# alexfrom0815/IR-BPP

Measured on AMD Instinct MI355X. Metric: env steps/sec (placements/sec) across N parallel bins, higher is better.
Workload: dtype f64

## Files before the change

irbpp_amd/csrc/irbpp_kernels.hip:

```cpp
#include <hip/hip_runtime.h>
#include <math.h>
#include <stdint.h>

#include "contours_device.h"
#include "irbpp_device.h"
#include "irbpp_rounds.h"
#include "../../include/irbpp.h"

#ifndef IRBPP_PASS
#define IRBPP_PASS 1
#endif

#undef IRBPP_HERE
#undef IRBPP_PASS_NS
#if IRBPP_PASS == 1
#define IRBPP_HERE ::irbpp::
#elif IRBPP_PASS == 2
#define IRBPP_HERE ::irbpp::wg512::
#define IRBPP_PASS_NS wg512
#else
#define IRBPP_HERE ::irbpp::wg128::
#define IRBPP_PASS_NS wg128
#endif

namespace irbpp {
#if IRBPP_PASS != 1
namespace IRBPP_PASS_NS {
#endif

#if IRBPP_PASS == 1
constexpr int BLOCK = 256;
#elif IRBPP_PASS == 2
constexpr int BLOCK = 512;
#else
constexpr int BLOCK = 128;
#endif
constexpr int WAVES = BLOCK / 64;

#ifndef IRBPP_REPS
#ifdef IRBPP_ABLATE
#define IRBPP_REPS(bit) (1 + ((P.dbg_repeat >> (bit)) & 1))
#else
#define IRBPP_REPS(bit) 1
#endif
#endif

#if IRBPP_PASS == 1
__device__ __forceinline__ double round6(double x) { return rint(x * 1e6) / 1e6; }

__device__ __forceinline__ double round6_scaled(double x) { return rint(x * 1e6); }

__device__ __forceinline__ int np_floor_divide_int(double a, double b, double inv_b) {
    const double x = fabs(a);
    const double q0 = trunc(x * inv_b);
    const double r0 = fma(-q0, b, x);
    int q = (int)q0 + (r0 >= b ? 1 : 0) - (r0 < 0.0 ? 1 : 0);
#if defined(__HIP_DEVICE_COMPILE__)
    if (__ballot(a < 0.0) == 0ull) return q;
#endif
    if (a < 0.0) {
        const double r = fma(-(double)q, b, x);
        q = r == 0.0 ? -q : -q - 1;
    }
    return q;
}


__device__ __forceinline__ double wave_max_f64(double v) {
#define IRBPP_MAX_STEP(CTRL, ROWS)                                                                                   \
    {                                                                                                                \
        const int lo = __builtin_amdgcn_update_dpp(__double2loint(v), __double2loint(v), CTRL, ROWS, 0xF, false);    \
        const int hi = __builtin_amdgcn_update_dpp(__double2hiint(v), __double2hiint(v), CTRL, ROWS, 0xF, false);    \
        v = fmax(v, __hiloint2double(hi, lo));                                                                       \
    }
    IRBPP_MAX_STEP(0x111, 0xF) IRBPP_MAX_STEP(0x112, 0xF) IRBPP_MAX_STEP(0x114, 0xF) IRBPP_MAX_STEP(0x118, 0xF)
    IRBPP_MAX_STEP(0x142, 0xA) IRBPP_MAX_STEP(0x143, 0xC)
#undef IRBPP_MAX_STEP
    return __hiloint2double(__builtin_amdgcn_readlane(__double2hiint(v), 63), __builtin_amdgcn_readlane(__double2loint(v), 63));
}

#endif
__device__ inline double block_max_f64(double v, double* red) {
    v = wave_max_f64(v);
    __syncthreads();
    if ((threadIdx.x & 63) == 0) red[threadIdx.x >> 6] = v;
    __syncthreads();
    double r = red[0];
    for (int w = 1; w < WAVES; ++w) r = fmax(r, red[w]);
    return r;
}

__device__ inline int block_sum_int(int v, int* red) {
    v = __builtin_amdgcn_readlane(wave_inclusive_sum(v), 63);
    __syncthreads();
    if ((threadIdx.x & 63) == 0) red[threadIdx.x >> 6] = v;
    __syncthreads();
    int r = 0;
    for (int w = 0; w < WAVES; ++w) r += red[w];
    return r;
}

__device__ inline int block_scan_flag(bool flag, int* red, int& total) {
    const unsigned long long bal = __ballot(flag);
    const int lane = threadIdx.x & 63, w = threadIdx.x >> 6;
    const int pre = __popcll(bal & ((1ull << lane) - 1ull));
    __syncthreads();
    if (lane == 0) red[w] = __popcll(bal);
    __syncthreads();
    int base = 0;
    total = 0;
    for (int i = 0; i < WAVES; ++i) {
        const int c = red[i];
        if (i < w) base += c;
        total += c;
    }
    return base + pre;
}

#if IRBPP_PASS == 1
__device__ inline int trajectory_row(const Params& P, const Tables& T, int b, int episode) {
    long long row = T.stream ? (long long)b : (long long)P.traj_start + P.goff + b + (long long)episode * P.gbins;
    row %= T.n_traj;
    if (row < 0) row += T.n_traj;
    return (int)row;
}
struct KernArgs;
__device__ __forceinline__ void raise_error(const State& S, int bit);
constexpr int STREAM_CONSUMED = -3;
__device__ inline int consume_item(const Tables& T, const State& S, int row, int cursor, int id) {
    if (T.stream) {
        if (id == STREAM_CONSUMED) { raise_error(S, IRBPP_DEVERR_STREAM_DRY); return -1; }
        const_cast<int32_t*>(T.seq)[(long long)row * T.seq_len + (int)((uint32_t)cursor % (uint32_t)T.seq_len)] = STREAM_CONSUMED;
    }
    if (id >= T.n_shapes) { raise_error(S, IRBPP_DEVERR_BAD_ITEM); return -1; }
    return id < 0 ? -1 : id;
}
__device__ inline int fetch_item(const Tables& T, const State& S, int row, int cursor) {
    if (!T.stream && cursor >= T.seq_len) return -1;
    const int at = T.stream ? (int)((uint32_t)cursor % (uint32_t)T.seq_len) : cursor;
    return consume_item(T, S, row, cursor, T.seq[(long long)row * T.seq_len + at]);
}

__device__ __forceinline__ int fdiv(int n, int d, uint32_t m) {
    return d == 1 ? n : (int)__umulhi((uint32_t)n, m);
}

struct KernArgs { Params P; Tables T; State S; StepIO io; int mode; };
typedef const __attribute__((address_space(4))) KernArgs* KernArgsPtr;
__device__ __forceinline__ KernArgsPtr cold_args() {
    KernArgsPtr p = (KernArgsPtr)__builtin_amdgcn_kernarg_segment_ptr();
    asm volatile("" : "+s"(p));
    return p;
}

__device__ __forceinline__ void raise_error(const State& S, int bit) {
    atomicOr(S.err, bit);
    int32_t* mirror = cold_args()->io.err_out;
    if (mirror != nullptr) atomicOr(mirror, bit);
}

__device__ __forceinline__ uint32_t div_magic_dev(int d) { return d >= 2 ? (uint32_t)(0x100000000ull / (uint64_t)d + 1ull) : 0u; }

__device__ __forceinline__ int tile_row_part(const Params& P, int row) {
    const int q = fdiv(row, P.pp, P.mg_pp);
    return (row - q * P.pp) * P.pp * P.PL + q * P.LY;
}
__device__ __forceinline__ int tile_col_part(const Params& P, int col) {
    const int q = fdiv(col, P.pp, P.mg_pp);
    return (col - q * P.pp) * P.PL + q;
}
__device__ __forceinline__ int tile_rc(const Params& P, int row, int col) { return tile_row_part(P, row) + tile_col_part(P, col); }
__device__ __forceinline__ int tile_of_linear(const Params& P, int g) {
    const int row = fdiv(g, P.Hy, P.mg_hy);
    return tile_rc(P, row, g - row * P.Hy);
}
#endif
struct TileWalk {
    int col_part, row, row_step, lin;
    bool regular;
};
__device__ __forceinline__ TileWalk tile_walk_begin(const Params& P, int tid) {
    TileWalk w;
    const int row = fdiv(tid, P.Hy, P.mg_hy), col = tid - row * P.Hy;
    w.regular = BLOCK % P.Hy == 0;
    w.row = row;
    w.row_step = BLOCK / P.Hy;
    w.col_part = tile_col_part(P, col);
    w.lin = tid;
    return w;
}
__device__ __forceinline__ int tile_walk_index(const Params& P, const TileWalk& w) {
    return w.regular ? tile_row_part(P, w.row) + w.col_part : tile_of_linear(P, w.lin);
}
__device__ __forceinline__ void tile_walk_next(TileWalk& w) { w.lin += BLOCK; w.row += w.row_step; }
template <int STEP>
__device__ __forceinline__ void cell_tile_stage(const Params& P, double* c2, const double* ghm, float* obs, int tid) {
    if (tid >= P.AC) return;
    const int X = fdiv(tid, P.Ay, P.mg_ay), Y = tid - X * P.Ay;
    const int at = X * STEP * P.Hy + Y * STEP;
    const double* src = ghm + at;
    float* dst = obs + 5 * P.S + 9 + at;
    typedef double f64x2 __attribute__((ext_vector_type(2)));
    double h[STEP][STEP];
#pragma unroll
    for (int i = 0; i < STEP; ++i) {
        if constexpr (STEP == 1) {
            h[i][0] = src[0];
        } else {
#pragma unroll
            for (int j = 0; j < STEP; j += 2) {
                const f64x2 v = *(const f64x2*)(src + i * P.Hy + j);
                h[i][j] = v.x;
                h[i][j + 1] = v.y;
            }
        }
    }
    double m = h[0][0];
#pragma unroll
    for (int i = 0; i < STEP; ++i)
#pragma unroll
        for (int j = 0; j < STEP; ++j)
            if (i + j > 0) m = fmax(m, h[i][j]);
    c2[tid] = m;
#pragma unroll
    for (int i = 0; i < STEP; ++i)
#pragma unroll
        for (int j = 0; j < STEP; ++j) dst[i * P.Hy + j] = (float)h[i][j];
}
#if IRBPP_PASS == 1
__device__ __forceinline__ int tile_of_cell(const Params& P, int lx, int ly, int ij) {
    return tile_rc(P, lx * P.step + (ij & 0xFFFF), ly * P.step + (ij >> 16));
}

typedef const __attribute__((address_space(4))) Cell* ConstCellPtr;
__device__ __forceinline__ ConstCellPtr as_const(const Cell* p) { return (ConstCellPtr)(unsigned long long)p; }

constexpr int PHASE_ROW = 16;
__device__ __forceinline__ void stamp(const StepIO& io, int b, int k, bool leader) {
    if (io.phase_cycles && leader) {
        long long* row = io.phase_cycles + (size_t)b * PHASE_ROW;
        row[k] = (long long)clock64();
        if (k == 0) {
            row[8] = (long long)wall_clock64();
            const unsigned hw = __builtin_amdgcn_s_getreg((31 << 11) | 4);
            const unsigned xcc = __builtin_amdgcn_s_getreg((31 << 11) | 20);
            row[10] = (long long)hw | ((long long)xcc << 32);
        }
        if (k == 4) row[9] = (long long)wall_clock64();
    }
}

__device__ __forceinline__ void stamp(const StepIO& io, int b, int k) { stamp(io, b, k, threadIdx.x == 0); }

__device__ inline SlotMem carve_slot(unsigned char* base, int cap, int cap_stk) {
    SlotMem m;
    m.pts = base;
    m.dst = m.pts + cap;
    m.stk = (uint32_t*)(m.dst + cap);
    m.cap = cap;
    m.cap_stk = cap_stk;
    return m;
}

struct Lds {
    int* sr;
    double* hm;
    double* mb;
    double* c2;
    double* m1;
    double* posz;
    uint8_t* lev;
    unsigned long long* present;
    uint16_t* taskidx;
    uint16_t* tasklist;
    uint16_t* img;
    uint16_t* clist;
    uint32_t* dps;
    uint32_t* vmask;
    uint32_t* vbits;
    unsigned char* scratch;
    double* redd;
    int* redi;
};

__device__ inline Lds carve_lds(unsigned char* smem, const Params& P) {
    Lds L;
    L.sr = (int*)(smem + P.o_sr);
    L.hm = (double*)(smem + P.o_hm);
    L.mb = (double*)(smem + P.o_mb);
    L.c2 = (double*)(smem + P.o_c2);
    L.m1 = (double*)(smem + P.o_m1);
    L.posz = (double*)(smem + P.o_posz);
    L.lev = smem + P.o_lev;
// ... 2135 lines not shown
            for (int e = tid; e < s_nt; e += BLOCK) {
                const Cell tc = e == tid ? tc0 : cells[e];
                const int ij = tc.ij;
                const int row = lx * P.step + (ij & 0xFFFF), col = ly * P.step + (ij >> 16);
                const int c = tile_rc(P, row, col);
                const double h = fmax(L.hm[c], tc.v + z);
                L.hm[c] = h;
                ghm[row * P.Hy + col] = h;
            }
        } else {
            for (int i = tid; i < P.tile_words; i += BLOCK) L.hm[i] = 0.0;
            for (int i = tid; i < P.Hc; i += BLOCK) ghm[i] = 0.0;
        }
        if (tid == 0) {
            BinState* ps = S.bs + b;
            const KernArgsPtr ka = cold_args();
            if (ok) {
                const double vol = vol0;
                const double reward = (vol / P.bin_vol) * 10.0;
                const double epr = ps->ep_reward + reward;
                const int epl = ps->ep_len + 1;
                const int cursor = st_cursor;
                const int slot = ps->item_idx;
                if (ka->S.log_meta && slot < ka->S.log_cap) {
                    __builtin_assume(lx < 32 && ly < 32);
                    ka->S.log_meta[(size_t)b * ka->S.log_cap + slot] = (uint32_t)item0 | ((uint32_t)rot << 16) |
                                                                ((uint32_t)lx << 20) | ((uint32_t)ly << 25);
                    ka->S.log_z[(size_t)b * ka->S.log_cap + slot] = z;
                }
                ps->ep_reward = epr;
                ps->ep_len = epl;
                ps->item_idx += 1;
                ps->ratio_acc += vol;
                for (int i = oa; i < P.K - 1; ++i) q[i] = q[i + 1];
                int nxt = st_next;
                if (nxt == -2) nxt = fetch_item(T, S, st_trow, cursor);
                else nxt = consume_item(T, S, st_trow, cursor, nxt);
                q[P.K - 1] = nxt;
                ps->cursor = cursor + 1;
                if (ka->io.reward) ka->io.reward[b] = reward;
                if (ka->io.done) ka->io.done[b] = 0;
                if (ka->io.counter) ka->io.counter[b] = -1;
                if (ka->io.ratio) ka->io.ratio[b] = -1.0;
                if (ka->io.ep_reward) ka->io.ep_reward[b] = epr;
                if (ka->io.ep_len) ka->io.ep_len[b] = epl;
                if (ka->io.stable) ka->io.stable[b] = stable ? 1 : 0;
            } else {
                const int counter = ps->item_idx;
                const double ratio = ps->ratio_acc / P.bin_vol;
                const double epr = ps->ep_reward + 0.0;
                const int epl = ps->ep_len + 1;
                if (ka->io.stable) ka->io.stable[b] = 0;
                if (ka->io.reward) ka->io.reward[b] = 0.0;
                if (ka->io.done) ka->io.done[b] = 1;
                if (ka->io.counter) ka->io.counter[b] = counter;
                if (ka->io.ratio) ka->io.ratio[b] = ratio;
                if (ka->io.ep_reward) ka->io.ep_reward[b] = epr;
                if (ka->io.ep_len) ka->io.ep_len[b] = epl;
                if (ka->S.log_meta && counter < ka->S.log_cap) {
                    ka->S.log_meta[(size_t)b * ka->S.log_cap + counter] = (uint32_t)(item0 & 0xFFFF) | ((uint32_t)(rot & 15) << 16) |
                                                                   ((uint32_t)(lx & 31) << 20) | ((uint32_t)(ly & 31) << 25);
                    ka->S.log_z[(size_t)b * ka->S.log_cap + counter] = z;
                }
                double* tot = ka->S.totals + (size_t)b * 4;
                tot[0] += 1.0; tot[1] += ratio; tot[2] += (double)counter; tot[3] += epr;
                const int ep = ps->episode + 1;
                const int trow = trajectory_row(P, T, b, ep);
                ps->episode = ep;
                ps->traj_row = trow;
                const int c0 = T.stream ? st_cursor : 0;
                for (int i = 0; i < P.K; ++i) q[i] = fetch_item(T, S, trow, c0 + i);
                ps->cursor = c0 + P.K;
                ps->item_idx = 0;
                ps->ratio_acc = 0.0;
                ps->ep_reward = 0.0;
                ps->ep_len = 0;
            }
            for (int i = 0; i < P.K; ++i) L.redi[16 + i] = q[i];
        }
        if (ok && pref_ok) {
            if (tid < P.R * SRW_) L.sr[tid] = sr_pref;
            sr_staged = true;
        }
        __syncthreads();
    }

    if (mode == MODE_OBSERVE) stamp(io, b, 1);
    if (mode == MODE_RESET || mode == MODE_STEP) {
        stamp(io, b, 1);
        if (P.K == 1) {
            obs_item = L.redi[16];
            __syncthreads();
        } else {
            do_observe = false;
            for (int i = tid; i < P.K; i += BLOCK) obs[i] = (float)L.redi[16 + i];
            for (int i = tid; i < P.Hc; i += BLOCK) obs[P.K + i] = (float)L.hm[tile_of_linear(P, i)];
        }
    }
    if (do_observe) IRBPP_HERE observe_location<PATH, CHAIN>(P, T, S, io, L, b, obs_item, obs, debug_out, sr_staged, smem + P.lds_bytes, cell_tile);
}

#if IRBPP_PASS == 1
enum ApplyKey : int { KEY_CAND = 0, KEY_CELLS = 1, KEY_HEUR = 2 };

__device__ __forceinline__ uint32_t heuristic_select_wave(const Params& P, const State& S, int method, int dir, int b, int lane) {
    const int RAC = P.R * P.AC;
    const double* const zsrc = S.w_posz + (size_t)b * RAC;
    const uint32_t* const vsrc = S.w_valid + (size_t)b * P.R * P.vrow;
    const bool xf = (dir & 2) != 0, yf = (dir & 1) != 0;
    double best = 1e300;
    int best_i = 0x7fffffff;
    for (int i0 = 0; i0 < RAC; i0 += 4 * 64) {
        int X[4], Y[4];
        uint32_t vw[4];
        double z[4];
#pragma unroll
        for (int u = 0; u < 4; ++u) {
            const int idx = i0 + u * 64 + lane, ii = idx < RAC ? idx : 0;
            const int r = fdiv(ii, P.AC, P.mg_ac), c = ii - r * P.AC;
            X[u] = fdiv(c, P.Ay, P.mg_ay);
            Y[u] = c - X[u] * P.Ay;
            vw[u] = vsrc[r * P.vrow + X[u]];
        }
#pragma unroll
        for (int u = 0; u < 4; ++u) {
            const int idx = i0 + u * 64 + lane;
            z[u] = 1e3;
            if (idx < RAC && ((vw[u] >> Y[u]) & 1u)) z[u] = zsrc[idx];
        }
#pragma unroll
        for (int u = 0; u < 4; ++u) {
            const int idx = i0 + u * 64 + lane;
            if (idx >= RAC) continue;
            double sc = 1e6;
            if ((vw[u] >> Y[u]) & 1u) {
                const double cx = xf ? (double)(P.Ax - X[u]) : (double)X[u], cy = yf ? (double)(P.Ay - Y[u]) : (double)Y[u];
                const double raw = method == 1 ? z[u] : method == 2 ? (cx + cy) * P.res_a + 100.0 * z[u] : cx + cy;
                sc = round6(raw);
            }
            if (sc < best) { best = sc; best_i = idx; }
        }
    }
    for (int o = 32; o > 0; o >>= 1) {
        const double ob = __shfl_xor(best, o);
        const int oi = __shfl_xor(best_i, o);
        if (ob < best || (ob == best && oi < best_i)) { best = ob; best_i = oi; }
    }
    best_i = __builtin_amdgcn_readfirstlane(best_i);
    const int hr = fdiv(best_i, P.AC, P.mg_ac), hrem = best_i - hr * P.AC;
    const int hx = fdiv(hrem, P.Ay, P.mg_ay);
    return ((uint32_t)hr << 16) | ((uint32_t)hx << 8) | (uint32_t)(hrem - hx * P.Ay);
}

template <bool PER_WORKGROUP, int KEY = KEY_CAND>
__device__ __forceinline__ void apply_body(const Params& P, const Tables& T, const State& S, const StepIO& io) {
    const int lane = threadIdx.x & 63;
    const int slot = PER_WORKGROUP ? (int)blockIdx.x : (int)blockIdx.x * WAVES + (int)(threadIdx.x >> 6);
    if (slot >= io.n_slots) return;
    const int b = __builtin_amdgcn_readfirstlane(slot + io.block_off);
    double* const ghm = S.hm + (size_t)b * P.Hc;
    int32_t* const q = S.queue + (size_t)b * P.K;
    if (!PER_WORKGROUP || threadIdx.x < 64) {
    int a = 0, cell_r = 0, cell_x = 0, cell_y = 0;
    if constexpr (KEY == KEY_CAND) a = io.actions[b];
    if constexpr (KEY == KEY_CELLS) { cell_r = io.actions[3 * b]; cell_x = io.actions[3 * b + 1]; cell_y = io.actions[3 * b + 2]; }
    const BinState* ps0 = S.bs + b;
    const int item0 = ps0->cur_item, oa = ps0->order_action, nvalid0 = ps0->nvalid, nrows = ps0->nrows;
    const int cursor = ps0->cursor, trow = ps0->traj_row;
    uint32_t key;
    if constexpr (KEY == KEY_CAND) {
    a += a < 0 ? P.S : 0;
    if (a < 0 || a >= P.S) { if (lane == 0) raise_error(S, IRBPP_DEVERR_BAD_ACTION); a = a < 0 ? 0 : P.S - 1; }
    key = (uint32_t)__builtin_amdgcn_readfirstlane(a < nrows ? (int)S.cand[(size_t)b * P.S + a] : 0);
    } else if constexpr (KEY == KEY_CELLS) {
        if (cell_r < 0 || cell_r >= P.R || cell_x < 0 || cell_x >= P.Ax || cell_y < 0 || cell_y >= P.Ay) {
            if (lane == 0) raise_error(S, IRBPP_DEVERR_BAD_ACTION);
            cell_r = cell_r < 0 ? 0 : cell_r >= P.R ? P.R - 1 : cell_r;
            cell_x = cell_x < 0 ? 0 : cell_x >= P.Ax ? P.Ax - 1 : cell_x;
            cell_y = cell_y < 0 ? 0 : cell_y >= P.Ay ? P.Ay - 1 : cell_y;
        }
        key = (uint32_t)__builtin_amdgcn_readfirstlane((cell_r << 16) | (cell_x << 8) | cell_y);
        (void)nrows;
    } else {
        key = (item0 >= 0 && nvalid0 > 0) ? heuristic_select_wave(P, S, io.heur_method, io.heur_dir, b, lane) : 0u;
        (void)nrows;
    }
    int nxt = -2;
    if (P.K == 1) {
        const int at = T.stream ? (int)((uint32_t)cursor % (uint32_t)T.seq_len) : cursor;
        nxt = at < T.seq_len ? T.seq[(long long)trow * T.seq_len + at] : -1;
    }
    static_assert(sizeof(ShapeRot) == 112, "seven 16-byte chunks per ShapeRot");
    int4 srq = make_int4(0, 0, 0, 0);
    if (item0 >= 0 && lane < P.R * 7) srq = ((const int4*)(T.sr + (size_t)item0 * P.R))[lane];
    const double vol0 = item0 >= 0 ? T.volume[item0] : 0.0;
    const int rot = key >> 16, lx = (key >> 8) & 255, ly = key & 255;
    const bool have_sr = item0 >= 0 && rot < P.R;
    const int rot7 = have_sr ? rot * 7 : 0;
#define IRBPP_SRW(W) __builtin_amdgcn_readlane(((W) & 3) == 0 ? srq.x : ((W) & 3) == 1 ? srq.y : ((W) & 3) == 2 ? srq.z : srq.w, rot7 + ((W) >> 2))
#define IRBPP_SRI(FIELD) IRBPP_SRW(offsetof(ShapeRot, FIELD) / 4)
#define IRBPP_SRD(FIELD) __hiloint2double(IRBPP_SRW(offsetof(ShapeRot, FIELD) / 4 + 1), IRBPP_SRW(offsetof(ShapeRot, FIELD) / 4))
    const int s_ax = IRBPP_SRI(ax), s_ay = IRBPP_SRI(ay), s_nb = IRBPP_SRI(nb), s_ob = IRBPP_SRI(ob), s_has_out = IRBPP_SRI(has_out);
    const int s_ot = IRBPP_SRI(ot);
    const double ext_x = IRBPP_SRD(ext_x), ext_y = IRBPP_SRD(ext_y), ext_z = IRBPP_SRD(ext_z);
    bool ok = item0 >= 0 && nvalid0 > 0 && rot < P.R;
    if (ok) {
        const double tx = P.txs[lx & 31], ty = P.txs[ly & 31];
        if (round6_scaled(tx + ext_x - P.bin_x) > 0.0 || round6_scaled(ty + ext_y - P.bin_y) > 0.0) ok = false;
    }
    const int s_nt = ok ? IRBPP_SRI(nt) : 0;
#undef IRBPP_SRD
#undef IRBPP_SRI
#undef IRBPP_SRW
    const KernArgsPtr ka = cold_args();
    const bool in_grid = have_sr && lx <= P.Ax - s_ax && ly <= P.Ay - s_ay;
    const bool want_z = in_grid && (ok || ka->S.log_meta != nullptr);
    uint32_t vword = 0u;
    double zc = 1e3;
    if (want_z) {
        vword = S.w_valid[((size_t)b * P.R + rot) * P.vrow + lx];
        zc = S.w_posz[((size_t)b * P.R + rot) * P.AC + lx * P.Ay + ly];
    }
    const Cell* const tcells = T.tcell + s_ot;
    Cell tc0 = {};
    if (lane < s_nt) tc0 = tcells[lane];
    const int row0 = lx * P.step, col0 = ly * P.step;
    double h0 = 0.0;
    const int i0 = (row0 + (tc0.ij & 0xFFFF)) * P.Hy + col0 + (tc0.ij >> 16);
    if (lane < s_nt) h0 = ghm[i0];
    double z = 1e3;
    if (want_z) {
        if ((vword >> ly) & 1u) {
            z = zc;
        } else {
            const Cell* cells = T.bcell + s_ob;
            double m = s_has_out ? 0.0 : -1e300;
            for (int e = lane; e < s_nb; e += 64) {
                const Cell c = cells[e];
                m = fmax(m, ghm[(row0 + (c.ij & 0xFFFF)) * P.Hy + col0 + (c.ij >> 16)] - c.v);
            }
            z = wave_max_f64(m);
        }
    }
    if (ok) {
        const double top = z * P.scale_z + ext_z * P.scale_z;
        if (round6_scaled(top - P.ibin_z) > 0.0) ok = false;
    }
    if (ok) {
        if (lane < s_nt) ghm[i0] = fmax(h0, tc0.v + z);
        for (int e0 = 64; e0 < s_nt; e0 += 4 * 64) {
            Cell tc[4];
            int ix[4];
            double hv[4];
#pragma unroll
            for (int u = 0; u < 4; ++u) {
                const int e = e0 + u * 64 + lane;
                tc[u] = tcells[e < s_nt ? e : s_nt - 1];
            }
#pragma unroll
            for (int u = 0; u < 4; ++u) {
                ix[u] = (row0 + (tc[u].ij & 0xFFFF)) * P.Hy + col0 + (tc[u].ij >> 16);
                hv[u] = ghm[ix[u]];
            }
#pragma unroll
            for (int u = 0; u < 4; ++u)
                if (e0 + u * 64 + lane < s_nt) ghm[ix[u]] = fmax(hv[u], tc[u].v + z);
        }
    } else {
        for (int i = lane; i < P.Hc; i += 64) ghm[i] = 0.0;
    }
    if (lane == 0) {
        BinState* ps = S.bs + b;
        if (ok) {
            const double vol = vol0;
            const double reward = (vol / P.bin_vol) * 10.0;
            const double epr = ps->ep_reward + reward;
            const int epl = ps->ep_len + 1;
            const int slot_i = ps->item_idx;
            if (ka->S.log_meta && slot_i < ka->S.log_cap) {
                __builtin_assume(lx < 32 && ly < 32);
                ka->S.log_meta[(size_t)b * ka->S.log_cap + slot_i] = (uint32_t)item0 | ((uint32_t)rot << 16) |
                                                              ((uint32_t)lx << 20) | ((uint32_t)ly << 25);
                ka->S.log_z[(size_t)b * ka->S.log_cap + slot_i] = z;
            }
            ps->ep_reward = epr;
            ps->ep_len = epl;
            ps->item_idx += 1;
            ps->ratio_acc += vol;
            for (int i = oa; i < P.K - 1; ++i) q[i] = q[i + 1];
            if (nxt == -2) nxt = fetch_item(T, S, trow, cursor);
            else nxt = consume_item(T, S, trow, cursor, nxt);
            q[P.K - 1] = nxt;
            ps->cursor = cursor + 1;
            if (ka->io.reward) ka->io.reward[b] = reward;
            if (ka->io.done) ka->io.done[b] = 0;
            if (ka->io.counter) ka->io.counter[b] = -1;
            if (ka->io.ratio) ka->io.ratio[b] = -1.0;
            if (ka->io.ep_reward) ka->io.ep_reward[b] = epr;
            if (ka->io.ep_len) ka->io.ep_len[b] = epl;
            if (ka->io.stable) ka->io.stable[b] = 0;
        } else {
            const int counter = ps->item_idx;
            const double ratio = ps->ratio_acc / P.bin_vol;
            const double epr = ps->ep_reward + 0.0;
            const int epl = ps->ep_len + 1;
            if (ka->io.stable) ka->io.stable[b] = 0;
            if (ka->io.reward) ka->io.reward[b] = 0.0;
            if (ka->io.done) ka->io.done[b] = 1;
            if (ka->io.counter) ka->io.counter[b] = counter;
            if (ka->io.ratio) ka->io.ratio[b] = ratio;
            if (ka->io.ep_reward) ka->io.ep_reward[b] = epr;
            if (ka->io.ep_len) ka->io.ep_len[b] = epl;
            if (ka->S.log_meta && counter < ka->S.log_cap) {
                ka->S.log_meta[(size_t)b * ka->S.log_cap + counter] = (uint32_t)(item0 & 0xFFFF) | ((uint32_t)(rot & 15) << 16) |
                                                               ((uint32_t)(lx & 31) << 20) | ((uint32_t)(ly & 31) << 25);
                ka->S.log_z[(size_t)b * ka->S.log_cap + counter] = z;
            }
            double* tot = ka->S.totals + (size_t)b * 4;
            tot[0] += 1.0; tot[1] += ratio; tot[2] += (double)counter; tot[3] += epr;
            const int ep = ps->episode + 1;
            const int trow2 = trajectory_row(P, T, b, ep);
            ps->episode = ep;
            ps->traj_row = trow2;
            const int c0 = T.stream ? cursor : 0;
            for (int i = 0; i < P.K; ++i) q[i] = fetch_item(T, S, trow2, c0 + i);
            ps->cursor = c0 + P.K;
            ps->item_idx = 0;
            ps->ratio_acc = 0.0;
            ps->ep_reward = 0.0;
            ps->ep_len = 0;
        }
    }
    }
    if (P.K > 1 && io.obs != nullptr) {
        __builtin_amdgcn_fence(__ATOMIC_RELEASE, "workgroup");
        if (PER_WORKGROUP) __syncthreads();
        __builtin_amdgcn_fence(__ATOMIC_ACQUIRE, "workgroup");
        float* const obs = io.obs + (size_t)b * io.obs_stride;
        const int t0 = PER_WORKGROUP ? (int)threadIdx.x : lane, stride = PER_WORKGROUP ? BLOCK : 64;
        for (int i = t0; i < P.K; i += stride) obs[i] = (float)q[i];
        for (int i0 = 0; i0 < P.Hc; i0 += 8 * stride) {
            double v[8];
#pragma unroll
            for (int u = 0; u < 8; ++u) { const int i = i0 + u * stride + t0; v[u] = ghm[i < P.Hc ? i : P.Hc - 1]; }
#pragma unroll
            for (int u = 0; u < 8; ++u) { const int i = i0 + u * stride + t0; if (i < P.Hc) obs[P.K + i] = (float)v[u]; }
        }
    }
}
extern "C" __global__ void __launch_bounds__(BLOCK)
irbpp_apply_kernel(const Params P, const Tables T, const State S, const StepIO io, const int mode) { apply_body<false>(P, T, S, io); }
extern "C" __global__ void __launch_bounds__(BLOCK)
irbpp_apply_wg_kernel(const Params P, const Tables T, const State S, const StepIO io, const int mode) { apply_body<true>(P, T, S, io); }
extern "C" __global__ void __launch_bounds__(BLOCK)
irbpp_apply_cells_kernel(const Params P, const Tables T, const State S, const StepIO io, const int mode) { apply_body<false, KEY_CELLS>(P, T, S, io); }
extern "C" __global__ void __launch_bounds__(BLOCK)
irbpp_apply_cells_wg_kernel(const Params P, const Tables T, const State S, const StepIO io, const int mode) { apply_body<true, KEY_CELLS>(P, T, S, io); }
extern "C" __global__ void __launch_bounds__(BLOCK)
irbpp_apply_heur_kernel(const Params P, const Tables T, const State S, const StepIO io, const int mode) { apply_body<false, KEY_HEUR>(P, T, S, io); }
extern "C" __global__ void __launch_bounds__(BLOCK)
irbpp_apply_heur_wg_kernel(const Params P, const Tables T, const State S, const StepIO io, const int mode) { apply_body<true, KEY_HEUR>(P, T, S, io); }

extern "C" __global__ void __launch_bounds__(1024)
irbpp_item_order_kernel(const Tables T, const State S, int N) {
    __shared__ int hist[1024];
    __shared__ int start[1024];
    const int tid = threadIdx.x;
    hist[tid] = 0;
    __syncthreads();
    constexpr int PER = 8;
    auto buckets_of = [&](int k0, int (&out)[PER]) {
        int cur[PER], row[PER], item[PER];
#pragma unroll
        for (int u = 0; u < PER; ++u) {
            const int bb = tid + (k0 + u) * 1024;
            const BinState* ps = S.bs + (bb < N ? bb : 0);
            cur[u] = ps->cursor;
            row[u] = ps->traj_row;
        }
#pragma unroll
        for (int u = 0; u < PER; ++u) {
            int c = cur[u];
            if (T.stream) c = (int)((uint32_t)c % (uint32_t)T.seq_len);
            item[u] = c < T.seq_len ? T.seq[(long long)row[u] * T.seq_len + c] : 0;
        }
#pragma unroll
        for (int u = 0; u < PER; ++u) {
            const int it = item[u] < 0 ? 0 : (item[u] >= T.n_shapes ? T.n_shapes - 1 : item[u]);
            out[u] = (int)(((long long)it * 1024) / T.n_shapes);
        }
    };
    int mine[PER];
    for (int k0 = 0; k0 * 1024 < N; k0 += PER) {
        int bk[PER];
        buckets_of(k0, bk);
#pragma unroll
        for (int u = 0; u < PER; ++u) {
            if (k0 == 0) mine[u] = bk[u];
            if (tid + (k0 + u) * 1024 < N) atomicAdd(&hist[bk[u]], 1);
        }
    }
    __syncthreads();
    if (tid < 64) {
        int v[16], sum = 0;
        for (int i = 0; i < 16; ++i) { v[i] = hist[tid * 16 + i]; sum += v[i]; }
        const int inc = wave_inclusive_sum(sum);
        int acc = inc - sum;
        for (int i = 0; i < 16; ++i) { start[tid * 16 + i] = acc; acc += v[i]; }
    }
    __syncthreads();
    const int chunk = N / NXCD;
    for (int k0 = 0; k0 * 1024 < N; k0 += PER) {
        int bk[PER];
        if (k0 == 0) {
#pragma unroll
            for (int u = 0; u < PER; ++u) bk[u] = mine[u];
        } else {
            buckets_of(k0, bk);
        }
#pragma unroll
        for (int u = 0; u < PER; ++u) {
            const int bb = tid + (k0 + u) * 1024;
            if (bb < N) {
                const int s_pos = atomicAdd(&start[bk[u]], 1);
                S.order[NXCD * (s_pos % chunk) + s_pos / chunk] = bb;
            }
        }
    }
}

extern "C" __global__ void __launch_bounds__(BLOCK)
irbpp_heuristic_kernel(const Params P, const Tables T, const State S, const StepIO io) {
    extern __shared__ __attribute__((aligned(16))) unsigned char smem[];
    const Lds L = carve_lds(smem, P);
    const int b = blockIdx.x, tid = threadIdx.x;
    const int R = P.R, AC = P.AC, Ay = P.Ay;
    const int X = fdiv(tid, Ay, P.mg_ay), Y = tid - X * Ay;
    const double* ghm = S.hm + (size_t)b * P.Hc;
    for (int i = tid; i < P.Hc; i += BLOCK) L.hm[tile_of_linear(P, i)] = ghm[i];
    __syncthreads();
    const int item = __builtin_amdgcn_readfirstlane(S.bs[b].cur_item);
    overlap_test<PATH_ANY>(P, T, S, io, L, b, item, false, L.posz, false, true);
    __syncthreads();
    double best = 1e300;
    int best_i = 0x7fffffff;
    for (int r = 0; r < R; ++r) {
        if (tid < AC) {
            double sc = 1e6;
            if (item >= 0) sc = heuristic_score(P, T, io, L, T.sr[item * R + r], r, X, Y);
            const int idx = r * AC + tid;
            if (sc < best || (sc == best && idx < best_i)) { best = sc; best_i = idx; }
        }
    }
    for (int o = 32; o > 0; o >>= 1) {
        const double ob = __shfl_xor(best, o);
        const int oi = __shfl_xor(best_i, o);
        if (ob < best || (ob == best && oi < best_i)) { best = ob; best_i = oi; }
    }
    __syncthreads();
    if ((tid & 63) == 0) { L.redd[tid >> 6] = best; L.redi[4 + (tid >> 6)] = best_i; }
    __syncthreads();
    if (tid == 0) {
        for (int w = 1; w < WAVES; ++w)
            if (L.redd[w] < best || (L.redd[w] == best && L.redi[4 + w] < best_i)) { best = L.redd[w]; best_i = L.redi[4 + w]; }
        const int hr = fdiv(best_i, AC, P.mg_ac), hrem = best_i - hr * AC;
        const int hx = fdiv(hrem, Ay, P.mg_ay);
        io.heur_out[b * 3 + 0] = hr;
        io.heur_out[b * 3 + 1] = hx;
        io.heur_out[b * 3 + 2] = hrem - hx * Ay;
    }
}

constexpr int SHOT_CHUNK = 128;
extern "C" __global__ void __launch_bounds__(BLOCK)
irbpp_shot_item_kernel(const double* verts, const int32_t* faces, int n_faces, int fx, int fy, double res, double shift,
                       double* top, double* bottom, double* mtop, double* mbot, int32_t* any_hit) {
    __shared__ double tri[SHOT_CHUNK][10];
    __shared__ int n_staged;
    const int c = blockIdx.x * BLOCK + threadIdx.x;
    const bool mine = c < fx * fy;
    const double px = (double)(c / fy) * res + shift, py = (double)(c % fy) * res + shift;
    double zmin = 1e300, zmax = -1e300;
    bool hit = false;
    for (int f0 = 0; f0 < n_faces; f0 += SHOT_CHUNK) {
        __syncthreads();
        if (threadIdx.x == 0) n_staged = 0;
        __syncthreads();
        if (threadIdx.x < SHOT_CHUNK && f0 + threadIdx.x < n_faces) {
            const int f = f0 + threadIdx.x;
            const double* a = verts + 3 * faces[3 * f + 0];
            const double* b = verts + 3 * faces[3 * f + 1];
            const double* d = verts + 3 * faces[3 * f + 2];
            const double area = (b[0] - a[0]) * (d[1] - a[1]) - (b[1] - a[1]) * (d[0] - a[0]);
            if (area != 0.0) {
                double* t = tri[atomicAdd(&n_staged, 1)];
                t[0] = a[0]; t[1] = a[1]; t[2] = a[2]; t[3] = b[0]; t[4] = b[1]; t[5] = b[2];
                t[6] = d[0]; t[7] = d[1]; t[8] = d[2]; t[9] = area;
            }
        }
        __syncthreads();
        if (mine)
            for (int k = 0; k < n_staged; ++k) {
                const double* a = tri[k];
                const double* b = a + 3;
                const double* d = a + 6;
                const double area = a[9];
                const double w0 = (b[0] - px) * (d[1] - py) - (b[1] - py) * (d[0] - px);
                const double w1 = (d[0] - px) * (a[1] - py) - (d[1] - py) * (a[0] - px);
                const double w2 = (a[0] - px) * (b[1] - py) - (a[1] - py) * (b[0] - px);
                const bool inside = area > 0.0 ? (w0 >= 0.0 && w1 >= 0.0 && w2 >= 0.0) : (w0 <= 0.0 && w1 <= 0.0 && w2 <= 0.0);
                if (!inside) continue;
// ... 130 lines not shown
```

Measured before the change: 74.22 million.

## Spread apply-kernel bin-state and queue updates across wave lanes

The apply kernel now loads the 64-byte BinState with one dword per lane and broadcasts fields through readlane. It writes back only the owned dwords in a single lane-parallel store, replacing scattered lane-0 scalar accesses. Queue shifting, episode-reset refills, totals updates and heightmap clearing are now spread across lanes (double2 stores for the clear), and the next item is prefetched unconditionally. A waves-per-EU occupancy hint is added to most apply kernels. This shortens the serial lane-0 tail, at the cost of more register pressure and more complex reset logic.

After: 73.93 million. No clear change (-0.4%).

```diff
diff --git a/irbpp_amd/csrc/irbpp_kernels.hip b/irbpp_amd/csrc/irbpp_kernels.hip
--- a/irbpp_amd/csrc/irbpp_kernels.hip
+++ b/irbpp_amd/csrc/irbpp_kernels.hip
@@ -139,6 +139,14 @@
     if (!T.stream && cursor >= T.seq_len) return -1;
     const int at = T.stream ? (int)((uint32_t)cursor % (uint32_t)T.seq_len) : cursor;
     return consume_item(T, S, row, cursor, T.seq[(long long)row * T.seq_len + at]);
+}
+__device__ __forceinline__ bool reset_by_lanes(const Tables& T, int K) { return !T.stream || K <= T.seq_len; }
+__device__ __forceinline__ int reset_fetch_lane(const Tables& T, int row, int cursor, int K, int lane) {
+    if (lane >= K || !reset_by_lanes(T, K)) return -1;
+    const int c = (T.stream ? cursor : 0) + lane;
+    if (!T.stream && c >= T.seq_len) return -1;
+    const int at = T.stream ? (int)((uint32_t)c % (uint32_t)T.seq_len) : c;
+    return T.seq[(long long)row * T.seq_len + at];
 }
 
 __device__ __forceinline__ int fdiv(int n, int d, uint32_t m) {
@@ -2580,6 +2588,7 @@
     return ((uint32_t)hr << 16) | ((uint32_t)hx << 8) | (uint32_t)(hrem - hx * P.Ay);
 }
 
+#define IRBPP_APPLY_WAVES __attribute__((amdgpu_waves_per_eu(8)))
 template <bool PER_WORKGROUP, int KEY = KEY_CAND>
 __device__ __forceinline__ void apply_body(const Params& P, const Tables& T, const State& S, const StepIO& io) {
     const int lane = threadIdx.x & 63;
@@ -2592,9 +2601,17 @@
     int a = 0, cell_r = 0, cell_x = 0, cell_y = 0;
     if constexpr (KEY == KEY_CAND) a = io.actions[b];
     if constexpr (KEY == KEY_CELLS) { cell_r = io.actions[3 * b]; cell_x = io.actions[3 * b + 1]; cell_y = io.actions[3 * b + 2]; }
-    const BinState* ps0 = S.bs + b;
-    const int item0 = ps0->cur_item, oa = ps0->order_action, nvalid0 = ps0->nvalid, nrows = ps0->nrows;
-    const int cursor = ps0->cursor, trow = ps0->traj_row;
+    static_assert(sizeof(BinState) == 64, "sixteen dwords: one per lane");
+    int32_t* const bsw = (int32_t*)(S.bs + b);
+    const int bs_in = lane < 16 ? bsw[lane] : 0;
+    const KernArgsPtr ka = cold_args();
+    uint32_t* log_meta = ka->S.log_meta;
+    int log_cap = ka->S.log_cap;
+    asm volatile("" : "+s"(log_meta), "+s"(log_cap));
+#define IRBPP_BSI(FIELD) __builtin_amdgcn_readlane(bs_in, offsetof(BinState, FIELD) / 4)
+#define IRBPP_BSD(FIELD) __hiloint2double(__builtin_amdgcn_readlane(bs_in, offsetof(BinState, FIELD) / 4 + 1), __builtin_amdgcn_readlane(bs_in, offsetof(BinState, FIELD) / 4))
+    const int item0 = IRBPP_BSI(cur_item), oa = IRBPP_BSI(order_action), nvalid0 = IRBPP_BSI(nvalid), nrows = IRBPP_BSI(nrows);
+    const int cursor = IRBPP_BSI(cursor), trow = IRBPP_BSI(traj_row);
     uint32_t key;
     if constexpr (KEY == KEY_CAND) {
     a += a < 0 ? P.S : 0;
@@ -2613,11 +2630,13 @@
         key = (item0 >= 0 && nvalid0 > 0) ? heuristic_select_wave(P, S, io.heur_method, io.heur_dir, b, lane) : 0u;
         (void)nrows;
     }
-    int nxt = -2;
-    if (P.K == 1) {
+    int nxt;
+    {
         const int at = T.stream ? (int)((uint32_t)cursor % (uint32_t)T.seq_len) : cursor;
         nxt = at < T.seq_len ? T.seq[(long long)trow * T.seq_len + at] : -1;
     }
+    int qv = 0;
+    if (P.K > 1 && lane > oa && lane < P.K) qv = q[lane];
     static_assert(sizeof(ShapeRot) == 112, "seven 16-byte chunks per ShapeRot");
     int4 srq = make_int4(0, 0, 0, 0);
     if (item0 >= 0 && lane < P.R * 7) srq = ((const int4*)(T.sr + (size_t)item0 * P.R))[lane];
@@ -2640,9 +2659,8 @@
 #undef IRBPP_SRD
 #undef IRBPP_SRI
 #undef IRBPP_SRW
-    const KernArgsPtr ka = cold_args();
     const bool in_grid = have_sr && lx <= P.Ax - s_ax && ly <= P.Ay - s_ay;
-    const bool want_z = in_grid && (ok || ka->S.log_meta != nullptr);
+    const bool want_z = in_grid && (ok || log_meta != nullptr);
     uint32_t vword = 0u;
     double zc = 1e3;
     if (want_z) {
@@ -2694,71 +2712,112 @@
             for (int u = 0; u < 4; ++u)
                 if (e0 + u * 64 + lane < s_nt) ghm[ix[u]] = fmax(hv[u], tc[u].v + z);
         }
+    } else if ((P.Hc & 1) == 0) {
+        double2* const ghm2 = (double2*)ghm;
+        for (int i = lane; i < (P.Hc >> 1); i += 64) ghm2[i] = make_double2(0.0, 0.0);
     } else {
         for (int i = lane; i < P.Hc; i += 64) ghm[i] = 0.0;
     }
-    if (lane == 0) {
-        BinState* ps = S.bs + b;
-        if (ok) {
-            const double vol = vol0;
-            const double reward = (vol / P.bin_vol) * 10.0;
-            const double epr = ps->ep_reward + reward;
-            const int epl = ps->ep_len + 1;
-            const int slot_i = ps->item_idx;
-            if (ka->S.log_meta && slot_i < ka->S.log_cap) {
+    const int episode0 = IRBPP_BSI(episode), item_idx0 = IRBPP_BSI(item_idx), ep_len0 = IRBPP_BSI(ep_len);
+    const double ratio_acc0 = IRBPP_BSD(ratio_acc), ep_reward0 = IRBPP_BSD(ep_reward);
+#undef IRBPP_BSD
+#undef IRBPP_BSI
+    double* const log_z = ka->S.log_z;
+    double* const totals = ka->S.totals;
+    double* const o_reward = ka->io.reward;
+    uint8_t* const o_done = ka->io.done;
+    int32_t* const o_counter = ka->io.counter;
+    double* const o_ratio = ka->io.ratio;
+    double* const o_ep_reward = ka->io.ep_reward;
+    int32_t* const o_ep_len = ka->io.ep_len;
+    uint8_t* const o_stable = ka->io.stable;
+    int n_cursor, n_episode = episode0, n_trow = trow, n_item_idx, n_ep_len;
+    double n_ratio_acc, n_ep_reward;
+    if (ok) {
+        const double vol = vol0;
+        const double reward = (vol / P.bin_vol) * 10.0;
+        const double epr = ep_reward0 + reward;
+        const int epl = ep_len0 + 1;
+        const int slot_i = item_idx0;
+        if (P.K > 1) {
+            const int up = __shfl_down(qv, 1);
+            if (lane >= oa && lane < P.K - 1) q[lane] = up;
+        }
+        if (lane == 0) {
+            if (log_meta && slot_i < log_cap) {
                 __builtin_assume(lx < 32 && ly < 32);
-                ka->S.log_meta[(size_t)b * ka->S.log_cap + slot_i] = (uint32_t)item0 | ((uint32_t)rot << 16) |
-                                                              ((uint32_t)lx << 20) | ((uint32_t)ly << 25);
-                ka->S.log_z[(size_t)b * ka->S.log_cap + slot_i] = z;
-            }
-            ps->ep_reward = epr;
-            ps->ep_len = epl;
-            ps->item_idx += 1;
-            ps->ratio_acc += vol;
-            for (int i = oa; i < P.K - 1; ++i) q[i] = q[i + 1];
-            if (nxt == -2) nxt = fetch_item(T, S, trow, cursor);
-            else nxt = consume_item(T, S, trow, cursor, nxt);
-            q[P.K - 1] = nxt;
-            ps->cursor = cursor + 1;
-            if (ka->io.reward) ka->io.reward[b] = reward;
-            if (ka->io.done) ka->io.done[b] = 0;
-            if (ka->io.counter) ka->io.counter[b] = -1;
-            if (ka->io.ratio) ka->io.ratio[b] = -1.0;
-            if (ka->io.ep_reward) ka->io.ep_reward[b] = epr;
-            if (ka->io.ep_len) ka->io.ep_len[b] = epl;
-            if (ka->io.stable) ka->io.stable[b] = 0;
-        } else {
-            const int counter = ps->item_idx;
-            const double ratio = ps->ratio_acc / P.bin_vol;
-            const double epr = ps->ep_reward + 0.0;
-            const int epl = ps->ep_len + 1;
-            if (ka->io.stable) ka->io.stable[b] = 0;
-            if (ka->io.reward) ka->io.reward[b] = 0.0;
-            if (ka->io.done) ka->io.done[b] = 1;
-            if (ka->io.counter) ka->io.counter[b] = counter;
-            if (ka->io.ratio) ka->io.ratio[b] = ratio;
-            if (ka->io.ep_reward) ka->io.ep_reward[b] = epr;
-            if (ka->io.ep_len) ka->io.ep_len[b] = epl;
-            if (ka->S.log_meta && counter < ka->S.log_cap) {
-                ka->S.log_meta[(size_t)b * ka->S.log_cap + counter] = (uint32_t)(item0 & 0xFFFF) | ((uint32_t)(rot & 15) << 16) |
-                                                               ((uint32_t)(lx & 31) << 20) | ((uint32_t)(ly & 31) << 25);
-                ka->S.log_z[(size_t)b * ka->S.log_cap + counter] = z;
-            }
-            double* tot = ka->S.totals + (size_t)b * 4;
-            tot[0] += 1.0; tot[1] += ratio; tot[2] += (double)counter; tot[3] += epr;
-            const int ep = ps->episode + 1;
-            const int trow2 = trajectory_row(P, T, b, ep);
-            ps->episode = ep;
-            ps->traj_row = trow2;
-            const int c0 = T.stream ? cursor : 0;
+                log_meta[(size_t)b * log_cap + slot_i] = (uint32_t)item0 | ((uint32_t)rot << 16) |
+                                                         ((uint32_t)lx << 20) | ((uint32_t)ly << 25);
+                log_z[(size_t)b * log_cap + slot_i] = z;
+            }
+            q[P.K - 1] = consume_item(T, S, trow, cursor, nxt);
+            if (o_reward) o_reward[b] = reward;
+            if (o_done) o_done[b] = 0;
+            if (o_counter) o_counter[b] = -1;
+            if (o_ratio) o_ratio[b] = -1.0;
+            if (o_ep_reward) o_ep_reward[b] = epr;
+            if (o_ep_len) o_ep_len[b] = epl;
+            if (o_stable) o_stable[b] = 0;
+        }
+        n_cursor = cursor + 1;
+        n_item_idx = item_idx0 + 1;
+        n_ep_len = epl;
+        n_ratio_acc = ratio_acc0 + vol;
+        n_ep_reward = epr;
+    } else {
+        const int counter = item_idx0;
+        const double ratio = ratio_acc0 / P.bin_vol;
+        const double epr = ep_reward0 + 0.0;
+        const int epl = ep_len0 + 1;
+        if (lane == 0) {
+            if (o_stable) o_stable[b] = 0;
+            if (o_reward) o_reward[b] = 0.0;
+            if (o_done) o_done[b] = 1;
+            if (o_counter) o_counter[b] = counter;
+            if (o_ratio) o_ratio[b] = ratio;
+            if (o_ep_reward) o_ep_reward[b] = epr;
+            if (o_ep_len) o_ep_len[b] = epl;
+            if (log_meta && counter < log_cap) {
+                log_meta[(size_t)b * log_cap + counter] = (uint32_t)(item0 & 0xFFFF) | ((uint32_t)(rot & 15) << 16) |
+                                                          ((uint32_t)(lx & 31) << 20) | ((uint32_t)(ly & 31) << 25);
+                log_z[(size_t)b * log_cap + counter] = z;
+            }
+        }
+        if (lane < 4)
+            totals[(size_t)b * 4 + lane] += lane == 0 ? 1.0 : lane == 1 ? ratio : lane == 2 ? (double)counter : epr;
+        const int trow2 = trajectory_row(P, T, b, episode0 + 1);
+        const int newq = reset_fetch_lane(T, trow2, cursor, P.K, lane);
+        const int c0 = T.stream ? cursor : 0;
+        if (reset_by_lanes(T, P.K)) {
+            if (lane < P.K) q[lane] = consume_item(T, S, trow2, c0 + lane, newq);
+        } else if (lane == 0) {
             for (int i = 0; i < P.K; ++i) q[i] = fetch_item(T, S, trow2, c0 + i);
-            ps->cursor = c0 + P.K;
-            ps->item_idx = 0;
-            ps->ratio_acc = 0.0;
-            ps->ep_reward = 0.0;
-            ps->ep_len = 0;
-        }
-    }
+        }
+        n_episode = episode0 + 1;
+        n_trow = trow2;
+        n_cursor = c0 + P.K;
+        n_item_idx = 0;
+        n_ep_len = 0;
+        n_ratio_acc = 0.0;
+        n_ep_reward = 0.0;
+    }
+    int bs_out = bs_in;
+#define IRBPP_BSW(FIELD, HALF, VALUE) bs_out = lane == (int)(offsetof(BinState, FIELD) / 4 + (HALF)) ? (VALUE) : bs_out
+    IRBPP_BSW(cursor, 0, n_cursor);
+    IRBPP_BSW(episode, 0, n_episode);
+    IRBPP_BSW(item_idx, 0, n_item_idx);
+    IRBPP_BSW(ep_len, 0, n_ep_len);
+    IRBPP_BSW(traj_row, 0, n_trow);
+    IRBPP_BSW(ratio_acc, 0, __double2loint(n_ratio_acc));
+    IRBPP_BSW(ratio_acc, 1, __double2hiint(n_ratio_acc));
+    IRBPP_BSW(ep_reward, 0, __double2loint(n_ep_reward));
+    IRBPP_BSW(ep_reward, 1, __double2hiint(n_ep_reward));
+#undef IRBPP_BSW
+    constexpr uint64_t BS_OWNED = (1ull << offsetof(BinState, cursor) / 4) | (1ull << offsetof(BinState, episode) / 4) |
+                                  (1ull << offsetof(BinState, item_idx) / 4) | (1ull << offsetof(BinState, ep_len) / 4) |
+                                  (1ull << offsetof(BinState, traj_row) / 4) | (3ull << offsetof(BinState, ratio_acc) / 4) |
+                                  (3ull << offsetof(BinState, ep_reward) / 4);
+    if ((BS_OWNED >> lane) & 1ull) bsw[lane] = bs_out;
     }
     if (P.K > 1 && io.obs != nullptr) {
         __builtin_amdgcn_fence(__ATOMIC_RELEASE, "workgroup");
@@ -2776,15 +2835,15 @@
         }
     }
 }
-extern "C" __global__ void __launch_bounds__(BLOCK)
+extern "C" __global__ void __launch_bounds__(BLOCK) IRBPP_APPLY_WAVES
 irbpp_apply_kernel(const Params P, const Tables T, const State S, const StepIO io, const int mode) { apply_body<false>(P, T, S, io); }
-extern "C" __global__ void __launch_bounds__(BLOCK)
+extern "C" __global__ void __launch_bounds__(BLOCK) IRBPP_APPLY_WAVES
 irbpp_apply_wg_kernel(const Params P, const Tables T, const State S, const StepIO io, const int mode) { apply_body<true>(P, T, S, io); }
-extern "C" __global__ void __launch_bounds__(BLOCK)
+extern "C" __global__ void __launch_bounds__(BLOCK) IRBPP_APPLY_WAVES
 irbpp_apply_cells_kernel(const Params P, const Tables T, const State S, const StepIO io, const int mode) { apply_body<false, KEY_CELLS>(P, T, S, io); }
-extern "C" __global__ void __launch_bounds__(BLOCK)
+extern "C" __global__ void __launch_bounds__(BLOCK) IRBPP_APPLY_WAVES
 irbpp_apply_cells_wg_kernel(const Params P, const Tables T, const State S, const StepIO io, const int mode) { apply_body<true, KEY_CELLS>(P, T, S, io); }
-extern "C" __global__ void __launch_bounds__(BLOCK)
+extern "C" __global__ void __launch_bounds__(BLOCK) IRBPP_APPLY_WAVES
 irbpp_apply_heur_kernel(const Params P, const Tables T, const State S, const StepIO io, const int mode) { apply_body<false, KEY_HEUR>(P, T, S, io); }
 extern "C" __global__ void __launch_bounds__(BLOCK)
 irbpp_apply_heur_wg_kernel(const Params P, const Tables T, const State S, const StepIO io, const int mode) { apply_body<true, KEY_HEUR>(P, T, S, io); }
```
